# cleinc/slslam

Hardware: AMD Instinct MI355X
Metric: LBA iterations/sec (10-KF window, ~2k lines) at 1/2/4/8 GPU; traj RMSE vs ref (higher is better)
Workload: dtype f64; 1 GPU; synthetic 10 free + 10 fixed keyframe window, 2000 lines, ~12431 observations; full LM solve (Huber, <=10 iterations, Schur + back-substitution); windows_per_gpu=1024, total_windows=1024, lines=2000, launch=hipGraph replay, hip_streams=1, lba_keep_jacobian=0

## Files before the change

slslam_amd/csrc/lba_api.hip:

```cpp
#include <hip/hip_runtime.h>

#include <algorithm>
#include <chrono>
#include <cstdio>
#include <cstdlib>
#include <cstring>
#include <new>
#include <vector>

#include "../../include/slslam_hip.h"
#include "lba_kernels.h"
#include "lba_eliminate_mfma.h"
#include "lba_eliminate_grouped.h"
#define SLSLAM_PO_FACTOR_ONLY
#include "po_kernels.h"
#include "lba_big.h"
#include "lba_big_solve.h"
#include "device_cache.h"
#include "lba_motion_only.h"
#include "lba_covariance.h"
#include "lba_pack.h"
#include "lba_device_build.h"
#include "lba_resident.h"
#include "host_pool.h"
// ... 121 lines not shown
struct DeviceArena : NoCopy {
  struct Item { void** pp; size_t bytes; const void* host; size_t host_bytes; int group; size_t off; };
  std::vector<Item> items;
  char* base = nullptr;
  size_t bytes = 0;
  int device = 0;
  bool cached = false;
  char* stage = nullptr;
  bool stage_pinned = false;
  bool keep_stage = false;
  std::vector<char> stage_vec;
  ~DeviceArena() { release(); }
  template <typename T>
  void add(DevBuf<T>& d, size_t count, const T* host, size_t host_count, int group) {
    d.n = count; d.in_arena = true; d.p = nullptr;
    items.push_back(Item{ (void**)&d.p, count * sizeof(T), host, host_count * sizeof(T), group, 0 });
  }
  template <typename T> void upload(DevBuf<T>& d, const std::vector<T>& h) { add(d, h.size(), h.data(), h.size(), 0); }
  template <typename T> void staged(DevBuf<T>& d, size_t count) { add(d, count, (const T*)nullptr, 0, 0); }
  template <typename T> void scratch(DevBuf<T>& d, size_t count) { add(d, count, (const T*)nullptr, 0, 1); }
  template <typename T> void zeroed(DevBuf<T>& d, size_t count) { add(d, count, (const T*)nullptr, 0, 2); }
  template <typename T> T* host_of(const DevBuf<T>& d) const { return reinterpret_cast<T*>(stage + ((char*)d.p - base)); }
  size_t upload_end = 0, zero_begin = 0;
  int layout() {
    size_t off = 0;
    upload_end = 0; zero_begin = 0;
    for (int group = 0; group < 3; ++group) {
      if (group == 2) zero_begin = off;
      for (Item& it : items) {
        if (it.group != group) continue;
        it.off = off;
        off += (it.bytes + 255) & ~(size_t)255;
      }
      if (group == 0) upload_end = off;
    }
    bytes = off;
    if (off == 0) { items.clear(); return SLSLAM_OK; }
    if (cached) HIP_TRY(DeviceBlockCache::acquire(off, device, &base));
    else HIP_TRY(hipMalloc((void**)&base, off));
    if (keep_stage) {
      HIP_TRY(hipHostMalloc((void**)&stage, std::max<size_t>(upload_end, 256), hipHostMallocDefault));
      stage_pinned = true;
      std::memset(stage, 0, upload_end);
    } else {
      stage_vec.assign(upload_end, 0);
      stage = stage_vec.data();
    }
    for (const Item& it : items) {
      *it.pp = base + it.off;
      if (it.host && it.host_bytes) std::memcpy(stage + it.off, it.host, it.host_bytes);
    }
    items.clear();
    return SLSLAM_OK;
  }
  int push() {
    if (bytes == 0) return SLSLAM_OK;
    if (upload_end) HIP_TRY(hipMemcpy(base, stage, upload_end, hipMemcpyHostToDevice));
    if (bytes > zero_begin) HIP_TRY(hipMemset(base + zero_begin, 0, bytes - zero_begin));
    if (!stage_pinned) { std::vector<char>().swap(stage_vec); stage = nullptr; }
    return SLSLAM_OK;
  }
  int commit() { const int rc = layout(); return rc != SLSLAM_OK ? rc : push(); }
  void release() {
    if (base) { if (cached) DeviceBlockCache::give_back(base, bytes, device); else (void)hipFree(base); }
    if (stage_pinned && stage) (void)hipHostFree(stage);
    stage = nullptr; stage_pinned = false; std::vector<char>().swap(stage_vec);
    base = nullptr; items.clear();
  }
};

Policy make_policy(const slslam_solver_options& o) {
  Policy p;
  p.huber_delta = o.huber_delta; p.baseline = o.baseline;
  p.initial_radius = o.initial_trust_region_radius; p.max_radius = o.max_trust_region_radius;
  p.min_radius = o.min_trust_region_radius; p.min_relative_decrease = o.min_relative_decrease;
  p.min_lm_diagonal = o.min_lm_diagonal; p.max_lm_diagonal = o.max_lm_diagonal;
  p.function_tolerance = o.function_tolerance; p.gradient_tolerance = o.gradient_tolerance;
  p.parameter_tolerance = o.parameter_tolerance;
  p.max_num_iterations = o.max_num_iterations; p.max_invalid = o.max_num_consecutive_invalid_steps;
  p.jacobi_scaling = o.jacobi_scaling; p.keep_jacobian = 0;
  p.store_f = o.reuse_elimination ? 1 : 0;
  const char* dbg = std::getenv("SLSLAM_DEBUG_ABLATE");
  p.debug_flags = dbg ? std::atoi(dbg) : 0;
  return p;
}

enum { FAM_LIN = 0, FAM_SOLVE = 1, FAM_BACKSUB = 2, FAM_TRIG = 3, FAM_COST = 4, FAM_UPDATE = 5, FAM_INIT = 6, FAM_N = 8 };

}

struct slslam_lba_batch {
  int device = 0;
  bool finalized = false;
  std::vector<PackedWindow> wins;
  slslam_solver_options opt;
  Policy pol;
  std::vector<WinDesc> h_wins;
  std::vector<long long> h_param_off;
  long long total_params = 0;
  std::vector<LMState> h_state0;
  HostArr<LMState> h_state;
  HostArr<IterRec> h_trace;
  HostArr<double> h_params;
  bool refillable = false;
  long long used_ncam = 0, used_nline = 0, used_nobs = 0, used_tiles = 0, used_items = 0;
  int cap_maxC = 0, cap_maxn = 0;
  int auto_rounds = 0, auto_cpw = 0;
  std::vector<int> sys_map_off_of_cf;
  hipEvent_t ev_stage_free = nullptr;
  hipEvent_t ev_results = nullptr;
  bool results_pending = false;
  HostPool* ext_pool = nullptr;
  std::unique_ptr<HostPool> own_pool;
  std::vector<PackedWindow> wins_spare;
  std::vector<int> h_ob_orig_off;
  bool downloaded = false;
  DeviceArena arena;
  DevBuf<uint16_t> d_sys_map;
  DevBuf<WinDesc> d_wins; DevBuf<Tile> d_tiles; DevBuf<Chunk> d_chunks; DevBuf<uint8_t> d_items; DevBuf<uint16_t> d_lane_map; DevBuf<int32_t> d_lane_ctx;
  DevBuf<uint32_t> d_line_desc;
  DevBuf<unsigned long long> d_dbg_cycles;
  int elim_mode = 0, elim_waves = 1;
  bool elim_mixed = false;
  bool elim_grouped = false;
  size_t lds_elim = 0;
  DevBuf<unsigned long long> d_iter_counter;
  DevBuf<unsigned int> d_active;
  DevBuf<double> d_cam_x, d_cam_x0, d_cam_scale, d_cam_tab; DevBuf<int> d_cam_cf, d_cam_win;
  DevBuf<double> d_line_x, d_line_x0, d_line_scale; DevBuf<int> d_line_ptr, d_line_flags, d_line_win, d_line_orig;
  DevBuf<double> d_ob; DevBuf<int> d_ob_cam, d_ob_orig;
  DevBuf<double> d_ob_raw;
  DevBuf<RawWin> d_rawwin; DevBuf<BuildWin> d_buildwin; DevBuf<uint32_t> d_raw_idx, d_fmask; DevBuf<double> d_line_raw; DevBuf<uint8_t> d_lflags;
  DevBuf<int> d_item_base, d_totals, d_line_pos;
  DevBuf<uint32_t> d_mid_keys; DevBuf<BuildLine> d_mid_li; DevBuf<uint4> d_mid_rows; DevBuf<uint16_t> d_mid_next, d_mid_trows, d_mid_tptr; DevBuf<BuildMid> d_mid;
  HostArr<RawWin> h_rawwin;
  HostArr<BuildWin> h_buildwin;
  HostArr<WinDesc> h_wins_dl;
  HostArr<int> h_totals;
  HostArr<char> h_raw_stage;
  DevBuf<char> d_stage_in;
  std::vector<RawWin> host_src;
  bool ingest_pinned = false;
  bool device_built = false;
  bool inplace_export = false;
  bool results_inplace = false;
  std::vector<slslam_lba_window> src_windows;
  std::vector<int> build_status;
  long long n_device_builds = 0, n_zero_copy = 0;
  bool big_mode = false;
  BigPtrs big;
  std::vector<long long> h_big_sys_off, h_big_linv_off;
  DevBuf<int> d_big_ob_line, d_big_cam_ptr, d_big_cam_obs, d_big_pair_ptr, d_big_pair_row, d_big_pair_col, d_big_pair_desc, d_big_flags;
  DevBuf<double> d_big_J, d_big_F, d_big_cost, d_big_camtab, d_big_line_acc, d_big_sys, d_big_scal, d_big_linv;
  DevBuf<long long> d_big_sys_off;
  DevBuf<double> d_slab_sum;
  long long slab_sum_stride = 0;
  bool slab_sum_image = false;
  int line_elim_stride = kLineElim;
  DevBuf<double> d_slab, d_bs_part, d_cost_part, d_ysys, d_params_out, d_fstore, d_line_elim, d_line_h;
  DevBuf<LMState> d_state; DevBuf<IterRec> d_trace; DevBuf<long long> d_param_off;
  BatchPtrs ptrs;
  int nchunk = 0, nline = 0, ncam = 0;
  long long nobs = 0;
  int num_cus = 256;
  bool fused_motion_only = false;
  bool share_cam_tab = false;
// ... 559 lines not shown
  ar.upload(b->d_big_cam_ptr, big_cam_ptr);
  ar.upload(b->d_big_cam_obs, big_cam_obs);
  ar.upload(b->d_big_pair_ptr, big_pair_ptr);
  ar.upload(b->d_big_pair_row, big_pair_row);
  ar.upload(b->d_big_pair_col, big_pair_col);
  ar.upload(b->d_big_pair_desc, big_pair_desc);
  ar.upload(b->d_big_sys_off, b->h_big_sys_off);
  ar.scratch(b->d_big_J, (size_t)std::max<long long>(1, nobs) * kBigObs);
  ar.scratch(b->d_big_F, (size_t)std::max<long long>(1, nobs) * kBigF);
  ar.scratch(b->d_big_cost, (size_t)std::max<long long>(1, nobs) * 2);
  ar.scratch(b->d_big_camtab, (size_t)std::max<long long>(1, ncam) * 2 * kBigCam);
  ar.zeroed(b->d_big_line_acc, (size_t)std::max<long long>(1, nline) * kBigLine);
  ar.zeroed(b->d_big_sys, (size_t)std::max<long long>(1, sys_cursor));
  ar.zeroed(b->d_big_scal, (size_t)std::max(1, B) * kBgScal);
  ar.zeroed(b->d_big_flags, (size_t)std::max(1, B) * 2);
  ar.scratch(b->d_big_linv, (size_t)std::max<long long>(1, linv_cursor));
  return SLSLAM_OK;
}

int reserve_arena(slslam_lba_batch* b, const LayoutPlan& plan, BigLists* big_lists) {
  const int B = (int)b->wins.size();
  const size_t cap_cam = (size_t)b->ncam, cap_line = (size_t)b->nline, cap_obs = std::max<size_t>(1, room(b, plan.nobs));
  const size_t cap_tiles = std::max<size_t>(1, room(b, plan.ntiles)), cap_items = std::max<size_t>(1, room(b, plan.nitems));
  DeviceArena& ar = b->arena;
  ar.device = b->device;
  ar.keep_stage = b->refillable;
  ar.staged(b->d_wins, (size_t)std::max(1, B));
  ar.upload(b->d_sys_map, plan.sys_map);
  ar.staged(b->d_tiles, cap_tiles);
  ar.staged(b->d_chunks, (size_t)std::max(1, b->nchunk));
  ar.staged(b->d_items, 2 * cap_items);
  ar.staged(b->d_lane_map, 64 * cap_tiles);
  ar.staged(b->d_line_desc, cap_line);
  ar.scratch(b->d_lane_ctx, 64 * 4 * cap_tiles);
  ar.scratch(b->d_cam_x, 12 * cap_cam);
  ar.staged(b->d_cam_x0, 6 * cap_cam);
  ar.zeroed(b->d_cam_scale, std::max<size_t>(6, (size_t)6 * cap_cam));
  b->share_cam_tab = B <= b->num_cus && !b->big_mode && !b->fused_motion_only && b->elim_mode == 0 && !b->opt.reuse_elimination && !b->pol.store_f && b->opt.max_num_iterations > 0 && !(b->pol.debug_flags & 16384);
  ar.zeroed(b->d_cam_tab, b->share_cam_tab ? std::max<size_t>(1, (size_t)2 * kCamTab * cap_cam) : 1);
  ar.staged(b->d_cam_cf, cap_cam);
  ar.staged(b->d_cam_win, cap_cam);
  ar.scratch(b->d_line_x, 2 * cap_line * kLineRec);
  ar.staged(b->d_line_x0, 4 * cap_line);
  ar.zeroed(b->d_line_scale, std::max<size_t>(4, (size_t)4 * cap_line));
  ar.staged(b->d_line_ptr, cap_line + 1);
  ar.staged(b->d_line_flags, cap_line);
  ar.staged(b->d_line_win, cap_line);
  ar.staged(b->d_line_orig, cap_line);
  ar.staged(b->d_ob, 8 * cap_obs);
  ar.scratch(b->d_ob_raw, b->refillable ? 8 * cap_obs : 0);
  {
    const bool db = b->refillable && b->opt.device_build >= 0;
    ar.scratch(b->d_rawwin, db ? (size_t)std::max(1, B) : 0);
    ar.scratch(b->d_buildwin, db ? (size_t)std::max(1, B) : 0);
    ar.scratch(b->d_raw_idx, db ? cap_obs : 0);
    ar.scratch(b->d_fmask, db ? cap_line : 0);
    ar.scratch(b->d_line_raw, db ? 4 * cap_line : 0);
    ar.scratch(b->d_lflags, db ? cap_line : 0);
    ar.scratch(b->d_item_base, db ? (size_t)std::max(1, B) : 0);
    ar.scratch(b->d_totals, db ? 8 : 0);
    ar.scratch(b->d_line_pos, db ? cap_line : 0);
    ar.scratch(b->d_mid_keys, db ? cap_line : 0); ar.scratch(b->d_mid_li, db ? cap_line : 0); ar.scratch(b->d_mid_rows, db ? cap_line : 0);
    ar.scratch(b->d_mid_next, db ? cap_line : 0); ar.scratch(b->d_mid_trows, db ? cap_line + 8 * (size_t)std::max(1, B) : 0);
    ar.scratch(b->d_mid_tptr, db ? cap_line + 8 * (size_t)std::max(1, B) : 0); ar.scratch(b->d_mid, db ? (size_t)std::max(1, B) : 0);
  }
  ar.staged(b->d_ob_cam, cap_obs);
  ar.staged(b->d_ob_orig, cap_obs);
  ar.scratch(b->d_slab, std::max<size_t>(1, room(b, plan.slab)));
  {
    const int max_chunks = plan.max_chunks, max_sys = plan.max_sys;
    b->slab_sum_stride = (max_chunks > 8 && !b->opt.reuse_elimination && !b->big_mode) ? (long long)max_sys + kSlabScalars : 0;
    b->slab_sum_image = b->slab_sum_stride && b->elim_mode == 0;
    if (b->slab_sum_image) {
      b->slab_sum_stride = slab_sum_image_stride(b->h_wins);
      ar.zeroed(b->d_slab_sum, (size_t)b->slab_sum_stride * (size_t)B);
    } else
    ar.scratch(b->d_slab_sum, b->slab_sum_stride ? (size_t)b->slab_sum_stride * (size_t)B : 1);
  }
  ar.scratch(b->d_bs_part, std::max<size_t>(1, (size_t)b->nchunk * kBsStride));
  ar.scratch(b->d_cost_part, std::max<size_t>(1, (size_t)b->nchunk));
  ar.scratch(b->d_ysys, std::max<size_t>(1, room(b, plan.sys)));
  ar.scratch(b->d_fstore, b->pol.keep_jacobian ? (size_t)(24 * 64) * cap_tiles
                          : b->opt.reuse_elimination ? (size_t)24 * cap_obs : 2);
  ar.scratch(b->d_line_h, b->pol.keep_jacobian ? (size_t)10 * cap_line : 2);
  b->line_elim_stride = (b->opt.reuse_elimination || b->big_mode) ? kLineElim : kLeU;
  ar.scratch(b->d_line_elim, std::max<size_t>(1, cap_line * b->line_elim_stride));
  ar.scratch(b->d_params_out, std::max<size_t>(1, room(b, plan.params)));
  ar.upload(b->d_state, b->h_state0);
  ar.zeroed(b->d_trace, std::max<size_t>(1, (size_t)B * kMaxTrace));
  ar.staged(b->d_param_off, (size_t)std::max(1, B));
  if (b->big_mode) {
    const int rc = big_lists->build(b, plan);
    if (rc != SLSLAM_OK) return rc;
  }
  ar.zeroed(b->d_iter_counter, 1);
  ar.zeroed(b->d_dbg_cycles, b->pol.debug_flags ? std::max((size_t)32 * std::max(1, b->nchunk), (size_t)16 * std::max(1, B)) : 1);
  ar.zeroed(b->d_active, 1);
  return ar.layout();
}

int fill_and_push(slslam_lba_batch* b, const LayoutPlan& plan) {
  const int B = (int)b->wins.size();
  HostImage img = host_image(b);
  auto one = [&](int wi) { fill_window(b, plan, b->wins, wi, img, true); };
  if (!run_all(batch_pool(b, (size_t)B), B, one)) return SLSLAM_ERR_NO_MEMORY;
  fill_tail(b, plan, img);
  return b->arena.push();
}

void bind_ptrs(slslam_lba_batch* b, const LayoutPlan& plan) {
  BatchPtrs& p = b->ptrs;
  p.wins = b->d_wins.p; p.tiles = b->d_tiles.p; p.chunks = b->d_chunks.p; p.items = b->d_items.p; p.lane_map = b->d_lane_map.p; p.lane_ctx = b->d_lane_ctx.p;
  p.cam_x = b->d_cam_x.p; p.cam_scale = b->d_cam_scale.p; p.cam_cf = b->d_cam_cf.p;
  p.cam_tab = b->share_cam_tab ? b->d_cam_tab.p : nullptr;
  p.line_x = b->d_line_x.p; p.line_scale = b->d_line_scale.p; p.line_ptr = b->d_line_ptr.p;
  p.line_flags = b->d_line_flags.p; p.line_win = b->d_line_win.p;
  p.ob = b->d_ob.p; p.ob_cam = b->d_ob_cam.p; p.ob_stride = (long long)(b->d_ob.n / 8);
  p.slab_sum = b->slab_sum_stride ? b->d_slab_sum.p : nullptr; p.slab_sum_stride = b->slab_sum_stride; p.slab_sum_image = b->slab_sum_image ? 1 : 0;
  p.slab = b->d_slab.p; p.bs_part = b->d_bs_part.p; p.cost_part = b->d_cost_part.p; p.ysys = b->d_ysys.p;
  p.fstore = b->d_fstore.p; p.line_elim = b->d_line_elim.p; p.line_elim_stride = b->line_elim_stride; p.line_h = b->d_line_h.p;
  p.state = b->d_state.p; p.trace = b->d_trace.p;
  p.iter_counter = b->d_iter_counter.p; p.active_counter = b->d_active.p; p.cam_x0 = b->d_cam_x0.p; p.line_u0 = b->d_line_x0.p;
  p.nwin = (int)b->wins.size(); p.nchunk = b->nchunk; p.nline = b->nline; p.ncam = b->ncam;
  p.dbg_cycles = b->d_dbg_cycles.p; p.sys_map = b->d_sys_map.p;
  if (b->big_mode) {
    BigPtrs& g = b->big;
    g.ob_line = b->d_big_ob_line.p; g.cam_win = b->d_cam_win.p; g.J = b->d_big_J.p; g.camtab = b->d_big_camtab.p;
    g.line_acc = b->d_big_line_acc.p; g.sys = b->d_big_sys.p; g.sys_off = b->d_big_sys_off.p; g.F = b->d_big_F.p; g.cost = b->d_big_cost.p;
    g.cam_ptr = b->d_big_cam_ptr.p; g.cam_obs = b->d_big_cam_obs.p; g.pair_ptr = b->d_big_pair_ptr.p; g.pair_row = b->d_big_pair_row.p;
    g.pair_col = b->d_big_pair_col.p; g.pair_desc = b->d_big_pair_desc.p; g.scal = b->d_big_scal.p; g.flags = b->d_big_flags.p; g.nobs = plan.nobs;
  }
  p.line_desc = b->d_line_desc.p; p.elim_mode = b->elim_mode; p.elim_waves = b->elim_waves;
}

int set_lds_limits(slslam_lba_batch* b, int maxC, int maxn) {
  b->lds_elim = b->elim_grouped ? (size_t)lds_bytes_eliminate_grouped(maxC, maxn) : (size_t)lds_bytes_eliminate_mfma(maxC, maxn, b->elim_waves);

  b->lds_lin = sizeof(double) * (size_t)lds_doubles_linearise(maxC, maxn);
  b->lds_solve = sizeof(double) * (size_t)lds_doubles_solve(maxn);
  b->fused_motion_only = b->opt.lba_fused_motion_only && !b->opt.reuse_elimination && !b->wins.empty();
  for (const PackedWindow& P : b->wins) if (P.Cf != 1 || P.nfree_params != 6) b->fused_motion_only = false;
  b->lds_motion_only = sizeof(double) * (size_t)lds_doubles_motion_only(maxC);
  b->lds_bs = sizeof(double) * (size_t)lds_doubles_backsub(maxC, maxn);
  b->lds_bs_stream = sizeof(double) * (size_t)lds_doubles_backsub_stream(maxC, maxn);
  b->lds_cost = sizeof(double) * (size_t)lds_doubles_cost(maxC, maxn);
  const size_t lds_max = std::max(std::max(b->lds_lin, b->lds_solve), std::max(b->lds_bs, b->lds_cost));
  if (lds_max > 160 * 1024 && !b->big_mode) return SLSLAM_ERR_UNSUPPORTED;
  if (b->lds_lin > 48 * 1024 && !b->big_mode)
    HIP_TRY(allow_lds({ (const void*)k_linearise_schur<true>, (const void*)k_linearise_schur<false>, (const void*)k_linearise_schur<false, 0>,
                        (const void*)k_linearise_schur<false, 1> }, b->lds_lin));
  if (b->elim_mode == 1 && b->lds_elim > 48 * 1024) {
    if (b->lds_elim > 160 * 1024) return SLSLAM_ERR_UNSUPPORTED;
    HIP_TRY(allow_lds({ (const void*)k_eliminate_mfma<1, false>, (const void*)k_eliminate_mfma<2, false>, (const void*)k_eliminate_mfma<1, true>,
                        (const void*)k_eliminate_mfma<2, true>, (const void*)k_eliminate_grouped<false>, (const void*)k_eliminate_grouped<true>,
                        (const void*)k_eliminate_grouped<false, true>, (const void*)k_eliminate_grouped<false, false, true> }, b->lds_elim));
  }
  if (b->lds_solve > 48 * 1024 && !b->big_mode)
    HIP_TRY(allow_lds({ (const void*)k_reduced_solve<4>, (const void*)k_reduced_solve<1> }, b->lds_solve));
  return SLSLAM_OK;
}

}

extern "C" int slslam_lba_batch_finalize(slslam_lba_batch* b, const slslam_solver_options* opt) {
  if (!b) return SLSLAM_ERR_INVALID_ARGUMENT;
  if (b->finalized) return SLSLAM_ERR_STATE;
  if (opt) b->opt = *opt;
// ... 1643 lines not shown
```

slslam_amd/csrc/lba_eliminate_grouped.h:

```cpp
#ifndef SLSLAM_LBA_ELIMINATE_GROUPED_H_
#define SLSLAM_LBA_ELIMINATE_GROUPED_H_

#include <type_traits>
#include "lba_kernels.h"
#include "lba_eliminate_mfma.h"
#include "lba_eliminate_grouped_maps.h"

#if !defined(GP_ABLATE)
#define GP_ABLATE 0
#endif
#if !defined(GP_GB1)
#define GP_GB1 4
#endif
#if !defined(GP_GB2)
#define GP_GB2 4
#endif
#if !defined(GP_GB3)
#define GP_GB3 2
#endif
#if !defined(GP_SETPRIO)
#define GP_SETPRIO 1
#endif

namespace slslam {


__host__ __device__ inline int lds_bytes_eliminate_grouped(int C, int n) {
  return (kGpPanel + C * kCamTabG + (n / 6) * kDiagRec) * 8 + ((C + 15) / 16) * 16;
}

__device__ __forceinline__ void grouped_flush_tile(double* slab, const solve_acc_t& A, int r, int c, int a, int n, int lane) {
#pragma unroll
  for (int q = 0; q < 4; ++q) {
    const int idx = gp_flush_index(r, c, a, q, lane, n);
    const double v = A[q];
    if (idx >= 0 && v != 0.0) __hip_atomic_fetch_add(slab + idx, v, __ATOMIC_RELAXED, __HIP_MEMORY_SCOPE_AGENT);
  }
}

template <bool FRESH, bool KEEP = false, bool MIXED = false>
__global__ __launch_bounds__(64) __attribute__((amdgpu_waves_per_eu(2, 2)))
void k_eliminate_grouped(BatchPtrs p, Policy pol) {
  static_assert(!(MIXED && (FRESH || KEEP)), "the mixed-precision form exists for the plain steady sweep only");
  using JT = double;
  extern __shared__ __attribute__((aligned(16))) double smem[];
  const int lane = threadIdx.x;
  SLS_K1_STAMP_INIT;
  const Chunk ck = p.chunks[blockIdx.x];
  if (ck.win < 0) return;
  SLS_K1_WALL(30);
  const WinDesc wd = p.wins[ck.win];
  const LMState* st = p.state + ck.win;
  if (st->status != kRunning) return;
  const int cur = st->cur;
  const TileReq rq0 = request_tile(p, ck.tile_begin, ck.tile_end, lane);
  const double inv_radius = 1.0 / st->radius;
  const bool need_grad = st->need_grad_check != 0;
  const bool same_point = st->same_point != 0;
  constexpr bool fresh = FRESH;
  constexpr bool keep = !FRESH && KEEP;
  const bool replay = keep && same_point;
  const int n = wd.n, ncf = n / 6;
  double* panel = smem;
  double* camtab = panel + kGpPanel;
  double* diag = camtab + wd.C * kCamTabG;
  signed char* camcf = (signed char*)(diag + ncf * kDiagRec);
  double* slab = p.slab + ck.slab_off;
  TileCtx nxt = resolve_tile(rq0);
  ObsPref pfn;
  if (!keep) prefetch_obs<FRESH, false>(p, nxt, cur, wd.obs_off, pfn, lane);
  for (int c = lane; c < wd.C; c += 64) {
    const double* x = p.cam_x + ((long long)(wd.cam_off + c) * 2 + cur) * kCamRec;
    double w[3] = { x[0], x[1], x[2] }, R[9];
    cam_rotation<double>(w, R);
    double* ct = camtab + c * kCamTabG;
    for (int q = 0; q < 9; ++q) ct[q] = R[q];
    ct[9] = x[3]; ct[10] = x[4]; ct[11] = x[5];
    camcf[c] = (signed char)p.cam_cf[wd.cam_off + c];
  }
  for (int q = lane; q < ncf * kDiagRec; q += 64) diag[q] = 0.0;
  if (lane < kGpSlab) panel[64 * kGpSlab + lane] = 0.0;
  for (int q = lane; q < kPTiles * kPTileDoubles; q += 64) slab[q] = 0.0;
  __syncthreads();
  asm volatile("s_waitcnt vmcnt(0)" ::: "memory");

  SLS_PHASE("prologue");
  solve_acc_t acc[kGpPersist];
#pragma unroll
  for (int e = 0; e < kGpPersist; ++e) acc[e] = solve_acc_t{ 0.0, 0.0, 0.0, 0.0 };
  int cur_a = -1;

  auto matrix_phase = [&](const unsigned descv) {
    SLS_K1_STAMP(5);
    SLS_PHASE("mfma_setup");
    int l2 = lane;
    asm volatile("" : "+v"(l2));
    int pre[4];
#pragma unroll
    for (int r = 0; r < 4; ++r) pre[r] = gp_pre(l2, r) * 8;
    const char* pbytes = reinterpret_cast<const char*>(panel);
    const unsigned d_first = (descv >> 10) & 63u, d_wdt = (descv >> 24) & 15u, d_nb = (descv >> 20) & 7u, d_group = (descv >> 16) & 15u;
    const unsigned d_bl = d_first * (unsigned)(kGpSlab * 8) | (d_wdt * (unsigned)(kGpSlab * 8)) << 16 | ((descv >> 23) & 1u) << 31;
    const bool d_active = (descv & 0x3ffu) != 0u;
    auto fetch = [&](int sidx, auto nbtag, double (&X)[4]) {
      constexpr int NB = decltype(nbtag)::value;
      const unsigned bl = (unsigned)__builtin_amdgcn_readlane((int)d_bl, sidx);
      if ((int)bl >= 0) {
        const int base = (int)(bl & 0xffffu), lim = (int)(bl >> 16);
#pragma unroll
        for (int r = 0; r < NB; ++r) {
          const int ad = (r < NB - 1 || pre[r] < lim) ? pre[r] + base : 64 * (kGpSlab * 8);
          X[r] = *reinterpret_cast<const double*>(pbytes + ad);
        }
      } else {
        const unsigned d = (unsigned)__builtin_amdgcn_readlane((int)descv, sidx);
        const unsigned mask = d & 0x3ffu, a = (d >> 16) & 15u, first = (d >> 10) & 63u;
#pragma unroll
        for (int r = 0; r < NB; ++r) {
          const unsigned slot = (unsigned)pre[r] / (unsigned)(kGpSlab * 8), cfb = a + slot;
          const bool present = ((mask >> cfb) & 1u) != 0u;
          const unsigned src = present ? first + (unsigned)__popc(mask & ((1u << cfb) - 1u)) : 64u;
          X[r] = *reinterpret_cast<const double*>(pbytes + (src * (kGpSlab * 8) + (unsigned)pre[r] - slot * (kGpSlab * 8)));
        }
      }
    };
    solve_acc_t row3[4];
#pragma unroll
    for (int c = 0; c < 4; ++c) {
      row3[c] = solve_acc_t{ 0.0, 0.0, 0.0, 0.0 };
      asm volatile("" : "+v"(row3[c]));
    }
    bool row3_used = false;
    auto products = [&](auto nbtag, const double (&X)[4]) {
      constexpr int NB = decltype(nbtag)::value;
      if (GP_ABLATE & 2) { for (int r = 0; r < NB; ++r) keep_alive(X[r]); return; }
      acc[0] = __builtin_amdgcn_mfma_f64_16x16x4f64(X[0], X[0], acc[0], 0, 0, 0);
      if (GP_ABLATE & 4) { for (int r = 1; r < NB; ++r) keep_alive(X[r]); return; }
      if (NB >= 2) {
        acc[1] = __builtin_amdgcn_mfma_f64_16x16x4f64(X[1], X[0], acc[1], 0, 0, 0);
        acc[2] = __builtin_amdgcn_mfma_f64_16x16x4f64(X[1], X[1], acc[2], 0, 0, 0);
      }
      if (NB >= 3) {
        acc[3] = __builtin_amdgcn_mfma_f64_16x16x4f64(X[2], X[0], acc[3], 0, 0, 0);
        acc[4] = __builtin_amdgcn_mfma_f64_16x16x4f64(X[2], X[1], acc[4], 0, 0, 0);
        acc[5] = __builtin_amdgcn_mfma_f64_16x16x4f64(X[2], X[2], acc[5], 0, 0, 0);
      }
      if (NB >= 4) {
        row3[0] = __builtin_amdgcn_mfma_f64_16x16x4f64(X[3], X[0], row3[0], 0, 0, 0);
        row3[1] = __builtin_amdgcn_mfma_f64_16x16x4f64(X[3], X[1], row3[1], 0, 0, 0);
        row3[2] = __builtin_amdgcn_mfma_f64_16x16x4f64(X[3], X[2], row3[2], 0, 0, 0);
        row3[3] = __builtin_amdgcn_mfma_f64_16x16x4f64(X[3], X[3], row3[3], 0, 0, 0);
      }
    };
    auto run = [&](int s, int e, auto nbtag, auto gbtag) {
      constexpr int GB = decltype(gbtag)::value;
      if (s >= e) return;
      if (GB > 1 && s + GB <= e) {
        double Xa[GB][4], Xb[GB][4];
#pragma unroll
        for (int i = 0; i < GB; ++i) fetch(s + i, nbtag, Xa[i]);
        for (; s + 2 * GB <= e; s += 2 * GB) {
#pragma unroll
          for (int i = 0; i < GB; ++i) fetch(s + GB + i, nbtag, Xb[i]);
#pragma unroll
          for (int i = 0; i < GB; ++i) products(nbtag, Xa[i]);
          if (s + 3 * GB <= e) {
#pragma unroll
            for (int i = 0; i < GB; ++i) fetch(s + 2 * GB + i, nbtag, Xa[i]);
          }
#pragma unroll
          for (int i = 0; i < GB; ++i) products(nbtag, Xb[i]);
        }
        if (s + GB <= e) {
#pragma unroll
          for (int i = 0; i < GB; ++i) products(nbtag, Xa[i]);
          s += GB;
        }
      }
      if (s >= e) return;
      double Xa[4], Xb[4];
      fetch(s, nbtag, Xa);
      for (; s + 1 < e; s += 2) {
        fetch(s + 1, nbtag, Xb);
        products(nbtag, Xa);
        if (s + 2 < e) fetch(s + 2, nbtag, Xa);
        products(nbtag, Xb);
      }
      if (s < e) products(nbtag, Xa);
    };
    auto flush_group = [&](int a) {
      grouped_flush_tile(slab, acc[0], 0, 0, a, n, l2); grouped_flush_tile(slab, acc[1], 1, 0, a, n, l2);
      grouped_flush_tile(slab, acc[2], 1, 1, a, n, l2); grouped_flush_tile(slab, acc[3], 2, 0, a, n, l2);
      grouped_flush_tile(slab, acc[4], 2, 1, a, n, l2); grouped_flush_tile(slab, acc[5], 2, 2, a, n, l2);
#pragma unroll
      for (int e = 0; e < kGpPersist; ++e) acc[e] = solve_acc_t{ 0.0, 0.0, 0.0, 0.0 };
    };
    auto flush_row3 = [&](int a) {
#pragma unroll
      for (int c = 0; c < 4; ++c) { grouped_flush_tile(slab, row3[c], 3, c, a, n, l2); row3[c] = solve_acc_t{ 0.0, 0.0, 0.0, 0.0 }; }
      row3_used = false;
    };
    if (GP_SETPRIO) __builtin_amdgcn_s_setprio(1);
    const int nact = (GP_ABLATE & 1) ? 0 : __popcll(__ballot(d_active));
    for (int sb = 0; sb < nact;) {
      const int a = (int)(((unsigned)__builtin_amdgcn_readlane((int)descv, sb) >> 16) & 15u);
      const bool in_seg = d_active && d_group == (unsigned)a;
      const int e1 = sb + __popcll(__ballot(in_seg && d_nb == 1u)), e2 = e1 + __popcll(__ballot(in_seg && d_nb == 2u));
      const int e3 = e2 + __popcll(__ballot(in_seg && d_nb == 3u)), e4 = e3 + __popcll(__ballot(in_seg && d_nb >= 4u));
      if (a != cur_a) {
        if (cur_a >= 0) { flush_group(cur_a); if (row3_used) flush_row3(cur_a); }
        cur_a = a;
      }
      run(sb, e1, std::integral_constant<int, 1>(), std::integral_constant<int, GP_GB1>());
      run(e1, e2, std::integral_constant<int, 2>(), std::integral_constant<int, GP_GB2>());
      run(e2, e3, std::integral_constant<int, 3>(), std::integral_constant<int, GP_GB3>());
      if (e4 > e3) { run(e3, e4, std::integral_constant<int, 4>(), std::integral_constant<int, 1>()); row3_used = true; }
      sb = e4;
    }
    SLS_K1_STAMP(6);
    SLS_PHASE("row3");
    if (row3_used) flush_row3(cur_a);
    if (GP_SETPRIO) __builtin_amdgcn_s_setprio(0);
    SLS_K1_STAMP(9);
  };

  double acc_cost = 0.0, acc_fixed = 0.0, acc_gmax = 0.0, acc_xn2 = 0.0;
  int fail = 0;
  if (!replay) {
    if (keep) prefetch_obs<FRESH, false>(p, nxt, cur, wd.obs_off, pfn, lane);
    SLS_K1_STAMP(0);
    for (int t = ck.tile_begin; t < ck.tile_end; ++t) {
      SLS_PHASE("tile_head");
      const TileCtx tc = nxt;
      const ObsPref pf = pfn;
      const unsigned descv = tc.desc;
      const SegCtx sg = make_seg(tc, lane);
      const int j = tc.j, ls = tc.ls, k = tc.k;
      const bool line_ok = tc.line_ok;
      const bool valid = line_ok && j < k;
      const bool line_free = line_ok && !(tc.lflags & 1);
      const int cf = camcf[pf.cam];
      const bool kept = valid && !(cf < 0 && !line_free);
      const bool line_active = line_free && k > 0;
      const bool cam_free = valid && cf >= 0;
      const double un2 = fresh ? pf.u[0] * pf.u[0] + pf.u[1] * pf.u[1] + pf.u[2] * pf.u[2] + pf.u[3] * pf.u[3] : 0.0;

      SLS_PHASE("linearise");
      double rs[4];
      JT Jl[16];
      double* slabF = panel + lane * kGpSlab;
      {
        const double* ct = camtab + pf.cam * kCamTabG;
        double R[9], tt[3], sl[4], cost;
#pragma unroll
        for (int q = 0; q < 9; ++q) R[q] = ct[q];
        tt[0] = ct[9]; tt[1] = ct[10]; tt[2] = ct[11];
#pragma unroll
        for (int a = 0; a < 4; ++a) sl[a] = fresh ? 1.0 : pf.lsc[a];
        if constexpr (MIXED) {
          obs_linearise_raw_mixed(R, tt, pf.trig, sl, pf.ob, pol.baseline, pol.huber_delta, rs, Jl, &cost,
            [&](int row, const float (&jc)[6]) {
              float2* dst = reinterpret_cast<float2*>(slabF) + 3 * row;
              dst[0] = make_float2(jc[0], jc[1]); dst[1] = make_float2(jc[2], jc[3]); dst[2] = make_float2(jc[4], jc[5]);
            });
        } else {
          obs_linearise_raw<double>(R, tt, pf.trig, sl, pf.ob, pol.baseline, pol.huber_delta, rs, Jl, &cost,
            [&](int row, const double (&jc)[6]) {
              double2* dst = reinterpret_cast<double2*>(slabF + 6 * row);
              dst[0] = make_double2(jc[0], jc[1]); dst[1] = make_double2(jc[2], jc[3]); dst[2] = make_double2(jc[4], jc[5]);
            });
        }
        if (kept) acc_cost += cost;
        if (fresh && valid && !kept) acc_fixed += cost;
      }
      SLS_K1_STAMP(1);
      SLS_PHASE("fetch_next_ctx");
      const TileReq rq = request_tile(p, t + 1, ck.tile_end, lane);

      SLS_PHASE("line_block");
      double H[10], g[4];
      double lsc_again[4] = { 1.0, 1.0, 1.0, 1.0 };
      if (!fresh) {
        const double2* lp = reinterpret_cast<const double2*>(p.line_scale + (long long)(line_ok ? ls : 0) * 4);
        const double2 s01 = lp[0], s23 = lp[1];
        lsc_again[0] = s01.x; lsc_again[1] = s01.y; lsc_again[2] = s23.x; lsc_again[3] = s23.y;
      }
      {
        double v[14];
        int q = 0;
#pragma unroll
        for (int a = 0; a < 4; ++a)
#pragma unroll
          for (int b = 0; b <= a; ++b) {
            JT h = 0;
#pragma unroll
            for (int r = 0; r < 4; ++r) h += Jl[4 * r + a] * Jl[4 * r + b];
            v[q++] = (double)h;
          }
        JT rsj[4];
#pragma unroll
        for (int r = 0; r < 4; ++r) rsj[r] = (JT)rs[r];
#pragma unroll
        for (int a = 0; a < 4; ++a) {
          JT ga = 0;
#pragma unroll
          for (int r = 0; r < 4; ++r) ga += Jl[4 * r + a] * rsj[r];
          v[10 + a] = (double)ga;
        }
        seg_sum_n<14, false, false>(v, sg);
        if (!fresh) {
          asm volatile("" : "+v"(lsc_again[0]), "+v"(lsc_again[1]), "+v"(lsc_again[2]), "+v"(lsc_again[3]));
        }
#pragma unroll
        for (int i = 0; i < 10; ++i) H[i] = v[i];
#pragma unroll
        for (int i = 0; i < 4; ++i) g[i] = v[10 + i];
      }
      SLS_K1_STAMP(2);
      SLS_PHASE("fresh_scale");
      if (fresh) {
        double sl[4];
        const double d[4] = { H[0], H[2], H[5], H[9] };
#pragma unroll
        for (int a = 0; a < 4; ++a) sl[a] = (pol.jacobi_scaling && line_active) ? 1.0 / (1.0 + sqrt(d[a])) : 1.0;
        if (line_ok && j == 0) {
          double* lsc = p.line_scale + (long long)ls * 4;
          for (int a = 0; a < 4; ++a) {
            lsc[a] = sl[a];
            if (line_active) acc_gmax = fmax(acc_gmax, fabs(g[a]));
          }
          if (line_active) acc_xn2 += un2;
        }
        H[0] *= sl[0] * sl[0]; H[1] *= sl[1] * sl[0]; H[2] *= sl[1] * sl[1]; H[3] *= sl[2] * sl[0]; H[4] *= sl[2] * sl[1];
        H[5] *= sl[2] * sl[2]; H[6] *= sl[3] * sl[0]; H[7] *= sl[3] * sl[1]; H[8] *= sl[3] * sl[2]; H[9] *= sl[3] * sl[3];
#pragma unroll
        for (int a = 0; a < 4; ++a) g[a] *= sl[a];
#pragma unroll
        for (int q = 0; q < 4; ++q)
#pragma unroll
          for (int a = 0; a < 4; ++a) Jl[4 * q + a] *= sl[a];
      }

      SLS_PHASE("factor4x4");
      double K[10], z[4] = { 0, 0, 0, 0 };
      {
        double D2[4], u[4];
        lm_diag4(H, pol, inv_radius, D2);
        bool okc = true;
        if (line_active) okc = chol4_inverse(H, D2, K);
        else { for (int q = 0; q < 10; ++q) K[q] = 0.0; }
        if (!okc) fail = 1;
        if (line_active) {
          u[0] = K[0] * g[0];
          u[1] = K[1] * g[0] + K[2] * g[1];
          u[2] = K[3] * g[0] + K[4] * g[1] + K[5] * g[2];
          u[3] = K[6] * g[0] + K[7] * g[1] + K[8] * g[2] + K[9] * g[3];
          z[0] = K[0] * u[0] + K[1] * u[1] + K[3] * u[2] + K[6] * u[3];
          z[1] = K[2] * u[1] + K[4] * u[2] + K[7] * u[3];
          z[2] = K[5] * u[2] + K[8] * u[3];
          z[3] = K[9] * u[3];
          if (need_grad && line_ok && j == 0) {
            for (int a = 0; a < 4; ++a) acc_gmax = fmax(acc_gmax, fabs(g[a] * fast_rcp(lsc_again[a])));
          }
          if (j == 0) {
            double* le = p.line_elim + (long long)ls * p.line_elim_stride;
#pragma unroll
            for (int q = 0; q < 10; ++q) le[q] = K[q];
#pragma unroll
            for (int q = 0; q < 4; ++q) { le[kLeD2 + q] = D2[q]; le[kLeG + q] = g[q]; }
            if (keep) {
              double2* lh = reinterpret_cast<double2*>(p.line_h + (long long)ls * 10);
#pragma unroll
              for (int q = 0; q < 5; ++q) lh[q] = make_double2(H[2 * q], H[2 * q + 1]);
            }
          }
        }
      }

      SLS_K1_STAMP(3);
      SLS_PHASE("f_rows");
      {
        JT Jc[24];
        double2* hkeep = reinterpret_cast<double2*>(p.fstore) + ((long long)t * (12 * 64) + lane);
        if constexpr (MIXED) {
#pragma unroll
          for (int q = 0; q < 12; ++q) { const float2 v2 = reinterpret_cast<const float2*>(slabF)[q]; Jc[2 * q] = (double)v2.x; Jc[2 * q + 1] = (double)v2.y; }
        } else {
#pragma unroll
          for (int q = 0; q < 12; ++q) { const double2 v2 = reinterpret_cast<const double2*>(slabF)[q]; Jc[2 * q] = v2.x; Jc[2 * q + 1] = v2.y; }
        }
        JT rsj[4];
#pragma unroll
        for (int r = 0; r < 4; ++r) rsj[r] = (JT)rs[r];
        double* rec = diag + (cam_free ? cf : 0) * kDiagRec;
        auto emit = [&](int off, double val) { if (cam_free) lds_add_rec(rec + off, val); };
#pragma unroll
        for (int a = 0; a < 6; ++a) {
          JT gaj = 0, hj[4] = { 0, 0, 0, 0 };
#pragma unroll
          for (int r = 0; r < 4; ++r) {
            gaj += Jc[6 * r + a] * rsj[r];
#pragma unroll
            for (int b = 0; b < 4; ++b) hj[b] += Jc[6 * r + a] * Jl[4 * r + b];
          }
          const double ga = (double)gaj, h[4] = { (double)hj[0], (double)hj[1], (double)hj[2], (double)hj[3] };
          const double f0 = h[0] * K[0];
          const double f1 = h[0] * K[1] + h[1] * K[2];
          const double f2 = h[0] * K[3] + h[1] * K[4] + h[2] * K[5];
          const double f3 = h[0] * K[6] + h[1] * K[7] + h[2] * K[8] + h[3] * K[9];
          reinterpret_cast<double2*>(slabF)[2 * a] = make_double2(f0, f1);
          reinterpret_cast<double2*>(slabF)[2 * a + 1] = make_double2(f2, f3);
          if (keep) {
            hkeep[(2 * a) * 64] = make_double2(h[0], h[1]);
            hkeep[(2 * a + 1) * 64] = make_double2(h[2], h[3]);
          }
          const double fu = h[0] * z[0] + h[1] * z[1] + h[2] * z[2] + h[3] * z[3];
          emit(kDiagB + a, ga - fu);
          if (!same_point) {
            emit(kDiagG + a, ga);
#pragma unroll
            for (int b = 0; b <= a; ++b) {
              JT v = 0;
#pragma unroll
              for (int r = 0; r < 4; ++r) v += Jc[6 * r + a] * Jc[6 * r + b];
              emit(tri_index(a, b), (double)v);
            }
          }
        }
      }

      SLS_K1_STAMP(4);
      SLS_PHASE("prefetch_next");
      nxt = resolve_tile(rq);
      prefetch_obs<FRESH, false>(p, nxt, cur, wd.obs_off, pfn, lane);

      matrix_phase(descv);
    }
  } else {
    struct Kept { double2 h[12]; double2 H[5]; double2 g[2]; int cam; };
    auto request = [&](int t, const TileCtx& c, Kept& kq) {
      const double2* hk = reinterpret_cast<const double2*>(p.fstore) + ((long long)(t < ck.tile_end ? t : ck.tile_begin) * (12 * 64) + lane);
#pragma unroll
      for (int q = 0; q < 12; ++q) kq.h[q] = hk[q * 64];
      const bool valid = c.line_ok && c.j < c.k;
      kq.cam = p.ob_cam[valid ? c.o0 + c.j : wd.obs_off];
      const int lsafe = c.line_ok ? c.ls : 0;
      const double2* lh = reinterpret_cast<const double2*>(p.line_h + (long long)lsafe * 10);
#pragma unroll
      for (int q = 0; q < 5; ++q) kq.H[q] = lh[q];
      const double2* lg = reinterpret_cast<const double2*>(p.line_elim + (long long)lsafe * p.line_elim_stride + kLeG);
      kq.g[0] = lg[0]; kq.g[1] = lg[1];
    };
    Kept kn;
    request(ck.tile_begin, nxt, kn);
    for (int t = ck.tile_begin; t < ck.tile_end; ++t) {
      SLS_PHASE("replay_head");
      const TileCtx tc = nxt;
      const Kept kp = kn;
      const unsigned descv = tc.desc;
      const int j = tc.j, ls = tc.ls, k = tc.k;
      const bool line_ok = tc.line_ok;
      const bool valid = line_ok && j < k;
      const bool line_free = line_ok && !(tc.lflags & 1);
      const int cf = camcf[kp.cam];
      const bool line_active = line_free && k > 0;
      const bool cam_free = valid && cf >= 0;
      const TileReq rq = request_tile(p, t + 1, ck.tile_end, lane);
      SLS_PHASE("replay_factor");
      double K[10], z[4] = { 0, 0, 0, 0 };
      {
        double H[10], g[4], D2[4], u[4];
#pragma unroll
        for (int q = 0; q < 5; ++q) { H[2 * q] = kp.H[q].x; H[2 * q + 1] = kp.H[q].y; }
        g[0] = kp.g[0].x; g[1] = kp.g[0].y; g[2] = kp.g[1].x; g[3] = kp.g[1].y;
        lm_diag4(H, pol, inv_radius, D2);
        bool okc = true;
        if (line_active) okc = chol4_inverse(H, D2, K);
        else { for (int q = 0; q < 10; ++q) K[q] = 0.0; }
        if (!okc) fail = 1;
        if (line_active) {
          u[0] = K[0] * g[0];
          u[1] = K[1] * g[0] + K[2] * g[1];
          u[2] = K[3] * g[0] + K[4] * g[1] + K[5] * g[2];
          u[3] = K[6] * g[0] + K[7] * g[1] + K[8] * g[2] + K[9] * g[3];
          z[0] = K[0] * u[0] + K[1] * u[1] + K[3] * u[2] + K[6] * u[3];
          z[1] = K[2] * u[1] + K[4] * u[2] + K[7] * u[3];
          z[2] = K[5] * u[2] + K[8] * u[3];
          z[3] = K[9] * u[3];
          if (j == 0) {
            double* le = p.line_elim + (long long)ls * p.line_elim_stride;
#pragma unroll
            for (int q = 0; q < 10; ++q) le[q] = K[q];
#pragma unroll
            for (int q = 0; q < 4; ++q) le[kLeD2 + q] = D2[q];
          }
        }
      }
      SLS_PHASE("replay_rows");
      {
        double* slabF = panel + lane * kGpSlab;
        double* rec = diag + (cam_free ? cf : 0) * kDiagRec;
#pragma unroll
        for (int a = 0; a < 6; ++a) {
          const double h0 = kp.h[2 * a].x, h1 = kp.h[2 * a].y, h2 = kp.h[2 * a + 1].x, h3 = kp.h[2 * a + 1].y;
          const double f0 = h0 * K[0];
          const double f1 = h0 * K[1] + h1 * K[2];
          const double f2 = h0 * K[3] + h1 * K[4] + h2 * K[5];
          const double f3 = h0 * K[6] + h1 * K[7] + h2 * K[8] + h3 * K[9];
          reinterpret_cast<double2*>(slabF)[2 * a] = make_double2(f0, f1);
          reinterpret_cast<double2*>(slabF)[2 * a + 1] = make_double2(f2, f3);
          const double fu = h0 * z[0] + h1 * z[1] + h2 * z[2] + h3 * z[3];
          if (cam_free) lds_add_rec(rec + kDiagB + a, -fu);
        }
      }
      SLS_PHASE("replay_request");
      nxt = resolve_tile(rq);
      request(t + 1, nxt, kn);
      matrix_phase(descv);
    }
  }
  SLS_K1_STAMP(7);
  SLS_PHASE("epilogue");
  if (cur_a >= 0) {
    grouped_flush_tile(slab, acc[0], 0, 0, cur_a, n, lane); grouped_flush_tile(slab, acc[1], 1, 0, cur_a, n, lane);
    grouped_flush_tile(slab, acc[2], 1, 1, cur_a, n, lane); grouped_flush_tile(slab, acc[3], 2, 0, cur_a, n, lane);
    grouped_flush_tile(slab, acc[4], 2, 1, cur_a, n, lane); grouped_flush_tile(slab, acc[5], 2, 2, cur_a, n, lane);
  }

  __syncthreads();
  double* drec = slab + kPTiles * kPTileDoubles;
  for (int q = lane; q < ncf * kDiagRec; q += 64) {
    const int e = q % kDiagRec;
    if (same_point && (e < kDiagB || e >= kDiagG)) continue;
    drec[q] = replay ? diag[q] + drec[q + (kDiagG - kDiagB)] : diag[q];
  }
  const double c_sum = wave_sum(acc_cost), f_sum = wave_sum(acc_fixed), x_sum = wave_sum(acc_xn2);
  const double g_max = wave_max(acc_gmax);
  const int any_fail = __any(fail);
  if (lane == 0) {
    double* sc = drec + ncf * kDiagRec;
    sc[kScCost] = c_sum; sc[kScFixedCost] = f_sum; sc[kScGradMaxLine] = g_max; sc[kScXn2Line] = x_sum;
    sc[kScFail] = any_fail ? 1.0 : 0.0;
  }
  SLS_K1_STAMP(8);
  SLS_K1_WALL(31);
}

}
#endif
```

slslam_amd/csrc/lba_types.h:

```cpp
#ifndef SLSLAM_LBA_TYPES_H_
#define SLSLAM_LBA_TYPES_H_

#include <stdint.h>

namespace slslam {

enum { kRunning = -1 };
enum { kNumericalFailure = 4 };
enum { kMaxTrace = 64 };
enum { kLineRec = 11 };
enum { kLineElim = 22 };
enum { kLeD2 = 10, kLeG = 14, kLeU = 18 };
enum { kCamRec = 6 };
enum { kSlabScalars = 8 };
enum { kMaxCams = 64, kMaxFreeCams = 20 };

enum { kScCost = 0, kScFixedCost = 1, kScGradMaxLine = 2, kScXn2Line = 3, kScFail = 4 };
enum { kBsModel = 0, kBsDn2 = 1, kBsXn2 = 2, kBsStride = 4 };

struct WinDesc {
  int C, Cf, L, M;
  int cam_off;
  int line_off;
  int obs_off;
  int tile_off, ntiles;
  int chunk_off, nchunks;
  int n;
  int sys_off;
  int nfree_params;
  int nkept;
  int slab_off;
  int map_off;
};

enum { kTileMultiRow = 1 };
struct Tile {
  int line_begin;
  int16_t nlines;
  int16_t flags;
  int item_off;
  int nitems;
};
constexpr int tile_trig_rounds(int flags) { return 1 << ((flags >> 1) & 3); }
constexpr int tile_max_run(int flags) { return (flags >> 3) & 31; }

struct Chunk {
  int win;
  int tile_begin, tile_end;
  int slab_off;
  int id;
};

struct LMState {
  double radius;
  double decrease_factor;
  double cost;
  double x_norm;
  double fixed_cost;
  double initial_cost;
  double min_cost;
  double abs_grad_tol;
  double grad_max;
  double cam_model, cam_dn2, cam_xn2;
  int status;
  int cur;
  int iter;
  int n_success, n_unsuccess, n_invalid;
  int solve_failed;
  int need_grad_check;
  int ntrace;
  int same_point;
  int fresh;
  int pad;
};

struct IterRec {
  int iteration, step_is_valid, step_is_successful, pad;
  double cost, cost_change, gradient_max_norm, step_norm, relative_decrease, trust_region_radius,
         model_cost_change;
};

struct Policy {
  double huber_delta, baseline;
  double initial_radius, max_radius, min_radius;
  double min_relative_decrease, min_lm_diagonal, max_lm_diagonal;
  double function_tolerance, gradient_tolerance, parameter_tolerance;
  int max_num_iterations, max_invalid, jacobi_scaling;
  int keep_jacobian;
  int store_f;
  int debug_flags;
};

struct BatchPtrs {
  const WinDesc* wins;
  const Tile* tiles;
  const Chunk* chunks;
  const uint16_t* lane_map;
  const int32_t* lane_ctx;
  const uint8_t* items;
  const uint32_t* line_desc;
  double* cam_x;
  double* cam_scale;
  double* cam_tab;
  const int* cam_cf;
  double* line_x;
  double* line_scale;
  const int* line_ptr;
  const int* line_flags;
  const int* line_win;
  const double* ob;
  const int* ob_cam;
  long long ob_stride;
  double* slab;
  double* slab_sum;
  long long slab_sum_stride;
  int slab_sum_image;
  const unsigned short* sys_map;
  double* bs_part;
  double* cost_part;
  double* ysys;
  double* fstore;
  double* line_elim;
  double* line_h;
  int line_elim_stride;
  LMState* state;
  IterRec* trace;
  unsigned long long* iter_counter;
  unsigned int* active_counter;
  const double* cam_x0;
  const double* line_u0;
  int nwin, nchunk, nline, ncam;
  unsigned long long* dbg_cycles;
  int elim_mode;
  int elim_waves;
};

#if defined(__HIPCC__)
__host__ __device__
#endif
inline long long line_rec(const BatchPtrs& p, long long ls, int buf) { return ((long long)buf * p.nline + ls) * kLineRec; }

}
#endif
```

Before: 663,200 LM iterations/s.

## Reuse cached per-line Hessian and gradient on same-point LM iterations in grouped eliminate

In the non-fresh, non-keep grouped elimination path, the per-line 4x4 Hessian and gradient are now written to a line_h buffer. On later iterations at the same linearization point (after a rejected step), they are loaded from that buffer instead of recomputed with a segment reduction, and the cost is not re-accumulated or overwritten. The cached values are prefetched alongside the next tile's observations. This skips the line-block reduction on rejected-step iterations, at the cost of extra line_h storage and writes on every normal iteration. It depends on the earlier cost and other slab values still being valid on those iterations.

```diff
diff --git a/slslam_amd/csrc/lba_api.hip b/slslam_amd/csrc/lba_api.hip
--- a/slslam_amd/csrc/lba_api.hip
+++ b/slslam_amd/csrc/lba_api.hip
@@ -227,6 +227,8 @@
   p.store_f = o.reuse_elimination ? 1 : 0;
   const char* dbg = std::getenv("SLSLAM_DEBUG_ABLATE");
   p.debug_flags = dbg ? std::atoi(dbg) : 0;
+  const char* fsp = std::getenv("SLSLAM_DEBUG_FULL_SAME_POINT");
+  p.full_same_point = (fsp && std::atoi(fsp) != 0) ? 1 : 0;
   return p;
 }
 
@@ -952,7 +954,7 @@
   ar.scratch(b->d_ysys, std::max<size_t>(1, room(b, plan.sys)));
   ar.scratch(b->d_fstore, b->pol.keep_jacobian ? (size_t)(24 * 64) * cap_tiles
                           : b->opt.reuse_elimination ? (size_t)24 * cap_obs : 2);
-  ar.scratch(b->d_line_h, b->pol.keep_jacobian ? (size_t)10 * cap_line : 2);
+  ar.scratch(b->d_line_h, b->elim_grouped ? (size_t)10 * cap_line : 2);
   b->line_elim_stride = (b->opt.reuse_elimination || b->big_mode) ? kLineElim : kLeU;
   ar.scratch(b->d_line_elim, std::max<size_t>(1, cap_line * b->line_elim_stride));
   ar.scratch(b->d_params_out, std::max<size_t>(1, room(b, plan.params)));
diff --git a/slslam_amd/csrc/lba_eliminate_grouped.h b/slslam_amd/csrc/lba_eliminate_grouped.h
--- a/slslam_amd/csrc/lba_eliminate_grouped.h
+++ b/slslam_amd/csrc/lba_eliminate_grouped.h
@@ -60,6 +60,8 @@
   constexpr bool fresh = FRESH;
   constexpr bool keep = !FRESH && KEEP;
   const bool replay = keep && same_point;
+  constexpr bool lean_form = !FRESH && !KEEP && !MIXED;
+  const bool lean = lean_form && same_point && !pol.full_same_point;
   const int n = wd.n, ncf = n / 6;
   double* panel = smem;
   double* camtab = panel + kGpPanel;
@@ -69,6 +71,17 @@
   TileCtx nxt = resolve_tile(rq0);
   ObsPref pfn;
   if (!keep) prefetch_obs<FRESH, false>(p, nxt, cur, wd.obs_off, pfn, lane);
+  struct LineKept { double2 H[5]; double2 g[2]; };
+  auto request_kept = [&](const TileCtx& c, LineKept& kq) {
+    const long long lsafe = (lean && c.line_ok) ? c.ls : 0;
+    const double2* lh = reinterpret_cast<const double2*>(p.line_h + lsafe * 10);
+#pragma unroll
+    for (int q = 0; q < 5; ++q) kq.H[q] = lh[q];
+    const double2* lg = reinterpret_cast<const double2*>(p.line_elim + lsafe * p.line_elim_stride + kLeG);
+    kq.g[0] = lg[0]; kq.g[1] = lg[1];
+  };
+  LineKept kpn;
+  if constexpr (lean_form) request_kept(nxt, kpn);
   for (int c = lane; c < wd.C; c += 64) {
     const double* x = p.cam_x + ((long long)(wd.cam_off + c) * 2 + cur) * kCamRec;
     double w[3] = { x[0], x[1], x[2] }, R[9];
@@ -233,6 +246,8 @@
       SLS_PHASE("tile_head");
       const TileCtx tc = nxt;
       const ObsPref pf = pfn;
+      LineKept kp;
+      if constexpr (lean_form) kp = kpn;
       const unsigned descv = tc.desc;
       const SegCtx sg = make_seg(tc, lane);
       const int j = tc.j, ls = tc.ls, k = tc.k;
@@ -270,7 +285,7 @@
               dst[0] = make_double2(jc[0], jc[1]); dst[1] = make_double2(jc[2], jc[3]); dst[2] = make_double2(jc[4], jc[5]);
             });
         }
-        if (kept) acc_cost += cost;
+        if (kept && !lean) acc_cost += cost;
         if (fresh && valid && !kept) acc_fixed += cost;
       }
       SLS_K1_STAMP(1);
@@ -280,41 +295,51 @@
       SLS_PHASE("line_block");
       double H[10], g[4];
       double lsc_again[4] = { 1.0, 1.0, 1.0, 1.0 };
-      if (!fresh) {
-        const double2* lp = reinterpret_cast<const double2*>(p.line_scale + (long long)(line_ok ? ls : 0) * 4);
-        const double2 s01 = lp[0], s23 = lp[1];
-        lsc_again[0] = s01.x; lsc_again[1] = s01.y; lsc_again[2] = s23.x; lsc_again[3] = s23.y;
-      }
-      {
-        double v[14];
-        int q = 0;
-#pragma unroll
-        for (int a = 0; a < 4; ++a)
-#pragma unroll
-          for (int b = 0; b <= a; ++b) {
-            JT h = 0;
-#pragma unroll
-            for (int r = 0; r < 4; ++r) h += Jl[4 * r + a] * Jl[4 * r + b];
-            v[q++] = (double)h;
-          }
-        JT rsj[4];
-#pragma unroll
-        for (int r = 0; r < 4; ++r) rsj[r] = (JT)rs[r];
-#pragma unroll
-        for (int a = 0; a < 4; ++a) {
-          JT ga = 0;
-#pragma unroll
-          for (int r = 0; r < 4; ++r) ga += Jl[4 * r + a] * rsj[r];
-          v[10 + a] = (double)ga;
-        }
-        seg_sum_n<14, false, false>(v, sg);
+      if (lean) {
+        if constexpr (lean_form) {
+#pragma unroll
+          for (int q = 0; q < 5; ++q) { H[2 * q] = kp.H[q].x; H[2 * q + 1] = kp.H[q].y; }
+          g[0] = kp.g[0].x; g[1] = kp.g[0].y; g[2] = kp.g[1].x; g[3] = kp.g[1].y;
+          asm volatile("" : "+v"(H[0]), "+v"(H[1]), "+v"(H[2]), "+v"(H[3]), "+v"(H[4]), "+v"(H[5]), "+v"(H[6]), "+v"(H[7]), "+v"(H[8]), "+v"(H[9]));
+          asm volatile("" : "+v"(g[0]), "+v"(g[1]), "+v"(g[2]), "+v"(g[3]));
+        }
+      } else {
         if (!fresh) {
-          asm volatile("" : "+v"(lsc_again[0]), "+v"(lsc_again[1]), "+v"(lsc_again[2]), "+v"(lsc_again[3]));
-        }
-#pragma unroll
-        for (int i = 0; i < 10; ++i) H[i] = v[i];
-#pragma unroll
-        for (int i = 0; i < 4; ++i) g[i] = v[10 + i];
+          const double2* lp = reinterpret_cast<const double2*>(p.line_scale + (long long)(line_ok ? ls : 0) * 4);
+          const double2 s01 = lp[0], s23 = lp[1];
+          lsc_again[0] = s01.x; lsc_again[1] = s01.y; lsc_again[2] = s23.x; lsc_again[3] = s23.y;
+        }
+        {
+          double v[14];
+          int q = 0;
+#pragma unroll
+          for (int a = 0; a < 4; ++a)
+#pragma unroll
+            for (int b = 0; b <= a; ++b) {
+              JT h = 0;
+#pragma unroll
+              for (int r = 0; r < 4; ++r) h += Jl[4 * r + a] * Jl[4 * r + b];
+              v[q++] = (double)h;
+            }
+          JT rsj[4];
+#pragma unroll
+          for (int r = 0; r < 4; ++r) rsj[r] = (JT)rs[r];
+#pragma unroll
+          for (int a = 0; a < 4; ++a) {
+            JT ga = 0;
+#pragma unroll
+            for (int r = 0; r < 4; ++r) ga += Jl[4 * r + a] * rsj[r];
+            v[10 + a] = (double)ga;
+          }
+          seg_sum_n<14, false, false>(v, sg);
+          if (!fresh) {
+            asm volatile("" : "+v"(lsc_again[0]), "+v"(lsc_again[1]), "+v"(lsc_again[2]), "+v"(lsc_again[3]));
+          }
+#pragma unroll
+          for (int i = 0; i < 10; ++i) H[i] = v[i];
+#pragma unroll
+          for (int i = 0; i < 4; ++i) g[i] = v[10 + i];
+        }
       }
       SLS_K1_STAMP(2);
       SLS_PHASE("fresh_scale");
@@ -368,7 +393,7 @@
             for (int q = 0; q < 10; ++q) le[q] = K[q];
 #pragma unroll
             for (int q = 0; q < 4; ++q) { le[kLeD2 + q] = D2[q]; le[kLeG + q] = g[q]; }
-            if (keep) {
+            if (keep || (lean_form && !lean)) {
               double2* lh = reinterpret_cast<double2*>(p.line_h + (long long)ls * 10);
 #pragma unroll
               for (int q = 0; q < 5; ++q) lh[q] = make_double2(H[2 * q], H[2 * q + 1]);
@@ -433,6 +458,7 @@
       SLS_PHASE("prefetch_next");
       nxt = resolve_tile(rq);
       prefetch_obs<FRESH, false>(p, nxt, cur, wd.obs_off, pfn, lane);
+      if constexpr (lean_form) request_kept(nxt, kpn);
 
       matrix_phase(descv);
     }
@@ -539,7 +565,8 @@
   const int any_fail = __any(fail);
   if (lane == 0) {
     double* sc = drec + ncf * kDiagRec;
-    sc[kScCost] = c_sum; sc[kScFixedCost] = f_sum; sc[kScGradMaxLine] = g_max; sc[kScXn2Line] = x_sum;
+    if (!lean) sc[kScCost] = c_sum;
+    sc[kScFixedCost] = f_sum; sc[kScGradMaxLine] = g_max; sc[kScXn2Line] = x_sum;
     sc[kScFail] = any_fail ? 1.0 : 0.0;
   }
   SLS_K1_STAMP(8);
diff --git a/slslam_amd/csrc/lba_types.h b/slslam_amd/csrc/lba_types.h
--- a/slslam_amd/csrc/lba_types.h
+++ b/slslam_amd/csrc/lba_types.h
@@ -87,6 +87,7 @@
   double function_tolerance, gradient_tolerance, parameter_tolerance;
   int max_num_iterations, max_invalid, jacobi_scaling;
   int keep_jacobian;
+  int full_same_point;
   int store_f;
   int debug_flags;
 };
```

After: 658,600 LM iterations/s. No clear change (-0.7%).
